# RNG65536/CUDA-volpath

Measured on AMD Instinct MI355X. Metric: Msamples/sec (WxHxspp) + achieved HBM GB/s, Julia 256^3 @ 800x600, higher is better.
Workload: dtype f32; 1 GPU; julia256_800x600_global_majorant; image=800x600, estimator=global_majorant, bound_brick=1, rng=philox2x32-7, parallelism=pixel-tiles x1

## Files before the change

cuda-volpath_amd/csrc/vp_device.h:

```cpp
#pragma once
#include <hip/hip_runtime.h>
#include <stdint.h>

#include "vp_math.h"

namespace vp
{
struct f3 { float x, y, z; };
VP_ARITH_BEGIN
__device__ __forceinline__ f3 mk3(float x, float y, float z) { return f3{x, y, z}; }
__device__ __forceinline__ f3 operator+(f3 a, f3 b) { return f3{a.x + b.x, a.y + b.y, a.z + b.z}; }
__device__ __forceinline__ f3 operator-(f3 a, f3 b) { return f3{a.x - b.x, a.y - b.y, a.z - b.z}; }
__device__ __forceinline__ f3 operator*(f3 a, f3 b) { return f3{a.x * b.x, a.y * b.y, a.z * b.z}; }
__device__ __forceinline__ f3 operator*(f3 a, float s) { return f3{a.x * s, a.y * s, a.z * s}; }
__device__ __forceinline__ f3 operator/(f3 a, float s) { return f3{a.x / s, a.y / s, a.z / s}; }
__device__ __forceinline__ float dot(f3 a, f3 b) { return a.x * b.x + a.y * b.y + a.z * b.z; }
__device__ __forceinline__ f3 cross(f3 a, f3 b)
{
    return f3{a.y * b.z - a.z * b.y, a.z * b.x - a.x * b.z, a.x * b.y - a.y * b.x};
}
__device__ __forceinline__ f3 normalize(f3 v) { return v * rsqrt_(dot(v, v)); }
__device__ __forceinline__ f3 normalize_ieee(f3 v) { return v * (1.0f / __builtin_sqrtf(dot(v, v))); }
__device__ __forceinline__ float max3(f3 v) { return fmaxf(fmaxf(v.x, v.y), v.z); }
__device__ __forceinline__ float min3(f3 v) { return fminf(fminf(v.x, v.y), v.z); }
VP_ARITH_END

#define VP_PI_F 3.1415926535897932384626422832795028841971f
constexpr float kPi     = VP_PI_F;
constexpr float kPi2    = VP_PI_F / 2.0f;
constexpr float k1Pi    = 1.0f / VP_PI_F;
constexpr float k1TwoPi = 1.0f / (VP_PI_F * 2.0f);
constexpr float kTwoPi  = VP_PI_F * 2.0f;
constexpr float k1TwoPiPi = 1.0f / VP_PI_F / (VP_PI_F * 2.0f);

struct ParamDev
{
    unsigned width, height;
    float    density, brightness;
    float    albedo[3];
    float    g;
    float    sigma_t[3];
};

struct SceneDev
{
    const uint2*         cells_u8;
    const float*         cells_f32;
    const unsigned char* bounds_u8;
    const float*         bounds_f32;
    const float*         opacity;
    const float*         opacity_cells;
    const float4*        env;
    int   nx, ny, nz, linear;
    int   cell_bricks;
    int   brick_shift, bnx, bny, bnz;
    int   env_w, env_h;
    float bmin[3], bmax[3], linv[3];
    float sun_dir[3], sun_power[3], sun_orig[3];
    float sun_cos;
    float cam[12];
    float cam_z;
    const float* env_cdf_y;
    const float* env_cdf_x;
    float        env_pdfnorm_alt;
};

__host__ __device__ __forceinline__ unsigned wang_hash(unsigned seed)
{
    seed = (seed ^ 61u) ^ (seed >> 16);
    seed *= 9u;
    seed = seed ^ (seed >> 4);
    seed *= 0x27d4eb2du;
    seed = seed ^ (seed >> 15);
    return seed;
}

struct RngSamplerH
{
    unsigned sx, sy;
    __device__ __forceinline__ void init(unsigned px, unsigned py, unsigned frame, unsigned, unsigned)
    {
        sx = wang_hash((px << 16) | py);
        sy = wang_hash(frame);
        word();
    }
    __device__ __forceinline__ unsigned word()
    {
        unsigned result = sx * 0x9e3779bbu;
        sy ^= sx;
        sx = ((sx << 26) | (sx >> 6)) ^ sy ^ (sy << 9);
        sy = (sx << 13) | (sx >> 19);
        return result;
    }
    __device__ __forceinline__ float next() { return u2f(0x3f800000u | (word() >> 9)) - 1.0f; }
    __device__ __forceinline__ float next_a() { return next(); }
    __device__ __forceinline__ float next_b() { return next(); }
    __device__ __forceinline__ void skip(unsigned n) { for (unsigned i = 0; i < n; i++) word(); }
    static constexpr bool kShadowSubstream = false;
    __device__ __forceinline__ unsigned enter_shadow(unsigned) { return 0u; }
    __device__ __forceinline__ void leave_shadow(unsigned) {}
    __device__ __forceinline__ void set_pair(unsigned) {}
    __device__ __forceinline__ void save(unsigned& a, unsigned& b) const { a = sx; b = sy; }
    __device__ __forceinline__ void load(unsigned a, unsigned b) { sx = a; sy = b; }
};

template <int ROUNDS>
struct RngPhiloxR
{
    unsigned pix, key, pair;
    unsigned w1;
    __device__ __forceinline__ void init(unsigned px, unsigned py, unsigned frame, unsigned key0, unsigned key1)
    {
        pix = (px << 16) | py; key = (frame ^ key0) + key1; pair = 0; w1 = 0;
    }
    __device__ __forceinline__ float next_a()
    {
        unsigned c0 = pair, c1 = pix, k = key;
#pragma unroll
        for (int r = 0; r < ROUNDS; r++)
        {
            unsigned long long p = (unsigned long long)0xD256D193u * c0;
            unsigned n0 = __builtin_amdgcn_bitop3_b32((unsigned)(p >> 32), k, c1, 0x96);
            c1 = (unsigned)p;
            c0 = n0;
            k += 0x9E3779B9u;
        }
        w1 = c1;
        pair++;
        return u2f(0x3f800000u | (c0 >> 9)) - 1.0f;
    }
    __device__ __forceinline__ float next_b() { return u2f(0x3f800000u | (w1 >> 9)) - 1.0f; }
    __device__ __forceinline__ void skip(unsigned n) { pair += n; }
    static constexpr bool kShadowSubstream = true;
    __device__ __forceinline__ unsigned enter_shadow(unsigned id) { const unsigned saved = pair; pair = 0x80000000u + (id << 20); return saved; }
    __device__ __forceinline__ void leave_shadow(unsigned saved) { pair = saved; }
    __device__ __forceinline__ void set_pair(unsigned n) { pair = n; }
    __device__ __forceinline__ void save(unsigned& a, unsigned& b) const { a = pair; b = 0u; }
    __device__ __forceinline__ void load(unsigned a, unsigned) { pair = a; }
};
typedef RngPhiloxR<10> RngPhilox;
typedef RngPhiloxR<7>  RngPhilox7;

VP_ARITH_BEGIN
#define VP_U8_TRI_SCALE 2.3374372e-10f
#define VP_U8_SCALE 0.003921569f

__device__ __forceinline__ f3 to_local(const SceneDev& S, f3 pos)
{
    return f3{(pos.x - S.bmin[0]) * S.linv[0], (pos.y - S.bmin[1]) * S.linv[1], (pos.z - S.bmin[2]) * S.linv[2]};
}

__device__ __forceinline__ void axis_linear(float pn, int n, int& i, float& fw)
{
    float xb = fma_(pn, (float)n, -0.5f);
    xb       = __builtin_fmaxf(xb, 0.0f);
    float fl = __builtin_floorf(xb);
    float fr = xb - fl;
    i        = (int)fl;
    fw       = __builtin_floorf(fma_(fr, 256.0f, 0.5f)) * (1.0f / 256.0f);
    i = i > n - 1 ? n - 1 : i;
}
__device__ __forceinline__ void axis_linear_f32(float pn, int n, int& i, float& fw, bool& low)
{
    float xb = fma_(pn, (float)n, -0.5f);
    float fl = __builtin_floorf(xb);
    float fr = xb - fl;
    i        = (int)fl;
    fw       = __builtin_floorf(fma_(fr, 256.0f, 0.5f)) * (1.0f / 256.0f);
    low      = i < 0;
    i        = i < 0 ? 0 : i;
    i        = i > n - 1 ? n - 1 : i;
}
__device__ __forceinline__ int axis_point(float pn, int n)
{
    int i = (int)__builtin_floorf(pn * (float)n);
    i     = i < 0 ? 0 : i;
    i     = i > n - 1 ? n - 1 : i;
    return i;
}

__device__ __forceinline__ float lerpf(float a, float b, float w) { return a * (1.0f - w) + b * w; }

__device__ __forceinline__ float filter_texels_u8(float t000, float t100, float t010, float t110, float t001, float t101, float t011, float t111,
                                                  float fx, float fy, float fz)
{
    float x00  = fma_(t100 - t000, fx, t000);
    float x10  = fma_(t110 - t010, fx, t010);
    float x01  = fma_(t101 - t001, fx, t001);
    float x11  = fma_(t111 - t011, fx, t011);
    float y0   = fma_(x10 - x00, fy, x00);
    float y1   = fma_(x11 - x01, fy, x01);
    float v    = fma_(y1 - y0, fz, y0);
    return v * (VP_U8_TRI_SCALE * 16777216.0f);
}
__device__ __forceinline__ float filter_cell_u8(uint2 c, float fx, float fy, float fz)
{
    float t000 = (float)(c.x & 0xffu), t100 = (float)((c.x >> 8) & 0xffu);
    float t010 = (float)((c.x >> 16) & 0xffu), t110 = (float)(c.x >> 24);
    float t001 = (float)(c.y & 0xffu), t101 = (float)((c.y >> 8) & 0xffu);
    float t011 = (float)((c.y >> 16) & 0xffu), t111 = (float)(c.y >> 24);
    float x00  = fma_(t100 - t000, fx, t000);
    float x10  = fma_(t110 - t010, fx, t010);
    float x01  = fma_(t101 - t001, fx, t001);
    float x11  = fma_(t111 - t011, fx, t011);
    float y0   = fma_(x10 - x00, fy, x00);
    float y1   = fma_(x11 - x01, fy, x01);
    float v    = fma_(y1 - y0, fz, y0);
    return v * (VP_U8_TRI_SCALE * 16777216.0f);
}

__device__ __forceinline__ size_t cell_index(const SceneDev& S, int i, int j, int k)
{
    if (S.cell_bricks)
    {
        const unsigned nbx = ((unsigned)S.nx + 3u) >> 2, nby = ((unsigned)S.ny + 3u) >> 2;
        const unsigned b   = ((unsigned)i >> 2) + nbx * (((unsigned)j >> 2) + nby * ((unsigned)k >> 2));
        return ((size_t)b << 6) | (size_t)((((unsigned)k & 3u) << 4) | (((unsigned)j & 3u) << 2) | ((unsigned)i & 3u));
    }
    return (size_t)((unsigned)i + __umul24((unsigned)S.nx, (unsigned)j + __umul24((unsigned)S.ny, (unsigned)k)));
}

template <bool QUANT>
__device__ __forceinline__ float sample_density01(const SceneDev& S, f3 pos)
{
    f3    p = to_local(S, pos);
    int   i, j, k;
    float fx, fy, fz;
    bool  lx = false, ly = false, lz = false;
    if (S.linear)
    {
        if (QUANT)
        {
            axis_linear(p.x, S.nx, i, fx);
            axis_linear(p.y, S.ny, j, fy);
            axis_linear(p.z, S.nz, k, fz);
        }
        else
        {
            axis_linear_f32(p.x, S.nx, i, fx, lx);
            axis_linear_f32(p.y, S.ny, j, fy, ly);
            axis_linear_f32(p.z, S.nz, k, fz, lz);
// ... 330 lines not shown
```

cuda-volpath_amd/csrc/vp_integrator.h:

```cpp
enum : int
{
    ST_DONE    = 0,
    ST_SETUP   = 1,
    ST_TRACK   = 2,
    ST_SHADOW  = 3,
    EV_SCATTER = 4,
    EV_NEE     = 5,
    EV_BG      = 6,
    EV_WRITE   = 7,
    EV_MIS     = 8,
    EV_HG      = 9
};

#ifndef VP_PAD_STEP
#define VP_PAD_STEP 0
#endif
#ifndef VP_PAD_FETCH
#define VP_PAD_FETCH 0
#endif
#ifndef VP_PAD_EOF
#define VP_PAD_EOF 0
#endif
#ifndef VP_PAD_SETUP
#define VP_PAD_SETUP 0
// ... 77 lines not shown
    const float c  = Ps + Pn;
    return Ps == 0.0f && sigma_t_prime * wdiv_(inv_sigma_t * c, Pn) == 1.0f;
}

__global__ void light_identity_k(ParamDev P, int local, const unsigned* mask, unsigned* flag)
{
    const unsigned b = threadIdx.x;
    if (local && !(mask[b >> 5] >> (b & 31u) & 1u)) return;
    if (!local && b) return;
    const float max_sig = max3(f3{P.sigma_t[0], P.sigma_t[1], P.sigma_t[2]});
    const float s       = hyperion_s(0 - 5);
    float sigma_t_prime;
    if (local)
    {
        const float reduction   = (1.0f - s) + s * (1.0f - P.g);
        const float cur_density = reduction * P.density;
        const float d_max       = fmaxf(0.0001f, (float)b * VP_U8_SCALE);
        sigma_t_prime           = max_sig * cur_density * d_max;
    }
    else
    {
        const float cur_density = (1.0f - s) * P.density + s * P.density * (1.0f - P.g);
        sigma_t_prime           = max_sig * cur_density;
    }
    const float inv_sigma_t = rcp_(sigma_t_prime);
    if (!(null_collision_in_empty_space(1.0f, sigma_t_prime, inv_sigma_t) == 1.0f)) atomicAnd(flag, 0u);
}

#ifndef VP_LOCAL_MIN_WAVES
#define VP_LOCAL_MIN_WAVES 6
#endif
constexpr int render_min_waves(int est, bool count, int ldsb, bool ach, bool mis, int trk, bool light, bool cancel)
{
    if (VP_MIN_WAVES > 1) return VP_MIN_WAVES;
    if (light) return count ? 5 : (est != EST_GLOBAL ? VP_LIGHT_LOCAL_MIN_WAVES : VP_LIGHT_MIN_WAVES);
    if (mis || ldsb == 1) return 1;
    if (count) return 4;
    if (est == EST_GLOBAL && trk == 0) return VP_GLOBAL_MIN_WAVES;
    if (trk) return 4;
    return (ach && !cancel) ? VP_LOCAL_MIN_WAVES : 5;
}
template <int EST, class RNG, bool QUANT, bool COUNT, int LDSB, bool ACH, bool MIS, int TRK, bool LIGHT = false, bool CANCEL = false>
__global__ __launch_bounds__(LDSB == 1 ? VP_BLOCK_LDS : VP_BLOCK, render_min_waves(EST, COUNT, LDSB, ACH, MIS, TRK, LIGHT, CANCEL))
void render_k(SceneDev S, LaunchDev L)
{
    __shared__ unsigned short lds_bounds[LDSB == 1 ? VP_LDS_BOUND_ENTRIES : 1];
    __shared__ unsigned lds_codes[LDSB == 2 ? VP_LDS_BOUND_ENTRIES / 16 : 1];
    if (LDSB == 2)
    {
        const uint4* src = reinterpret_cast<const uint4*>(L.bound_codes);
        uint4*       dst = reinterpret_cast<uint4*>(lds_codes);
        const int    n16 = (S.bnx * S.bny * S.bnz + 63) / 64;
        for (int w = threadIdx.x; w < n16; w += VP_BLOCK) dst[w] = src[w];
        __syncthreads();
    }
    if (LDSB == 1)
    {
        const uint4* src = reinterpret_cast<const uint4*>(S.bounds_u8);
        uint4*       dst = reinterpret_cast<uint4*>(lds_bounds);
        const int    n16 = (S.bnx * S.bny * S.bnz * 2 + 15) / 16;
        for (int w = threadIdx.x; w < n16; w += VP_BLOCK_LDS) dst[w] = src[w];
        __syncthreads();
    }
    constexpr unsigned KARG_L_   = ((sizeof(SceneDev) + alignof(LaunchDev) - 1) / alignof(LaunchDev)) * alignof(LaunchDev);
    constexpr unsigned KARG_WDS_ = (KARG_L_ + sizeof(LaunchDev) + 3) / 4;
    __shared__ __attribute__((aligned(16))) unsigned kargs_lds_[KARG_WDS_];
    {
        const unsigned* src = (const unsigned*)__builtin_amdgcn_kernarg_segment_ptr();
        for (unsigned w = threadIdx.x; w < KARG_WDS_; w += (LDSB == 1 ? VP_BLOCK_LDS : VP_BLOCK)) kargs_lds_[w] = src[w];
    }
    constexpr bool LOCAL = EST != EST_GLOBAL;
    constexpr bool TAB = TRK == 0 && LDSB != 1 && !LIGHT && !MIS;
    __shared__ __attribute__((aligned(16))) float coll_tab_[TAB ? VP_COLL_ROWS : 1][CR_WORDS];
    if (TAB && threadIdx.x < VP_COLL_ROWS)
        coll_row_fill(coll_tab_[threadIdx.x], (int)threadIdx.x, L.P.g, L.P.density, max3(f3{L.P.sigma_t[0], L.P.sigma_t[1], L.P.sigma_t[2]}), LOCAL);
    __syncthreads();
    auto coll_row = [&](int n) __attribute__((always_inline)) -> const float* {
        return TAB ? coll_tab_[n < 0 ? 0 : (n > VP_COLL_ROWS - 1 ? VP_COLL_ROWS - 1 : n)] : nullptr;
    };
    constexpr bool EARLY = RNG::kShadowSubstream && !MIS && !LIGHT;
    constexpr bool APPR = EST == EST_GLOBAL && TRK == 0 && !LIGHT && !MIS;
    constexpr bool APPR_L = EST == EST_DECOMP && TRK == 0 && !LIGHT && !MIS;
    constexpr bool EXITC = TRK == 0 && !MIS && !LIGHT && EST != EST_BOUNDED && (QUANT || EST == EST_GLOBAL);
    const ParamDev& P = L.P;
    const f3    sig_t     = f3{P.sigma_t[0], P.sigma_t[1], P.sigma_t[2]};
    const f3    sig_s     = sig_t * f3{P.albedo[0], P.albedo[1], P.albedo[2]};
    const float max_sig   = max3(sig_t);
    const float min_sig   = min3(sig_t);
    const float density   = P.density;

    int      st = ST_DONE;
    bool     exhausted = false;
    constexpr bool COLD = LDSB != 1 && !LIGHT;
    constexpr int  CS_  = COLD ? VP_BLOCK : 1;
    static_assert(!COLD || (LOCAL ? VP_LOCAL_MIN_WAVES : VP_GLOBAL_MIN_WAVES) * (14 * VP_BLOCK * 4 + KARG_WDS_ * 4 + VP_COLL_ROWS * CR_WORDS * 4 + (LDSB == 2 ? VP_LDS_BOUND_ENTRIES / 4 : 0)) <= VP_LDS_BYTES_PER_CU,
                  "cold per-path state: more workgroups per CU than the LDS holds -- lower VP_*_MIN_WAVES for this ARCH");
    __shared__ float cold_[COLD ? 14 : 1][CS_];
    float* const cold_p = &cold_[0][COLD ? threadIdx.x : 0];
    ColdF3<COLD, CS_>       rad(cold_p), pd(cold_p + 3 * CS_);
    ColdVal<float, COLD>    ph(cold_p + 6 * CS_), phase_g(cold_p + 7 * CS_);
    ColdVal<unsigned, COLD> item(cold_p + 8 * CS_);
    ColdVal<unsigned, COLD> px(cold_p + 9 * CS_), py(cold_p + 10 * CS_);
    ColdVal<int, COLD>      frame(cold_p + 11 * CS_);
    ColdVal<int, COLD>      nsc(cold_p + 12 * CS_);
    ColdVal<unsigned, COLD> rng_saved(cold_p + 13 * CS_);
    if (COLD) { rad = f3{0.0f, 0.0f, 0.0f}; pd = f3{0.0f, 0.0f, 0.0f}; ph = 0.0f; phase_g = 0.0f; item = 0u; px = 0u; py = 0u; frame = 0; nsc = 0; rng_saved = 0u; }
    RNG      rng;
    f3       ro = {}, rd = {};
    f3       inv_rd = {};
    f3       thr = {};
    int      seg = 0;
    float    dist = 0, t_end = 0;
    float    t_far = 0, distc = 0, inv_sigma = 0, inv_sigma_t = 0, sigma_t_prime = 0, sigma_c = 0;
    float    cur_density = 0, d_max = 0;
    f3       nee_a = {};
    int      terms = 0;
    f3       nee_c = {}, nee_t = {}, seg_o = {};
    int      nee_stage = 0;
    float    sh_inv_sigma = 0, sh_density = 0;
    float    sig_base = density;
    int      chan = 0;
    float    t_empty = 0.0f;
    float    t_clip = 1e30f;
    bool     ex_clear = false;
    unsigned long long c_load = 0, c_xtest = 0, c_xout = 0, c_xok = 0;
    unsigned zrun = 0;

    unsigned long long c_den = 0, c_bnd = 0, c_opa = 0, c_env = 0, c_sca = 0, c_smp = 0;
    unsigned long long d_iter = 0, d_act = 0, d_outer = 0, d_shadow = 0;
    constexpr bool PROF = COUNT && VP_PROFILE_BLOCKS;
    unsigned long long t_slow = 0, t_fast = 0, t_mark = PROF ? __builtin_amdgcn_s_memtime() : 0ull;
    enum { B_SETUP, B_HALF, B_LOOK, B_EXIT, B_SCATTER, B_NEE, B_HG, B_BG, B_WRITE, B_REFILL, B_GSETUP, B_FETCH, B_ZERO, B_ZERO_SH, B_EXITT, B_NBLK };
    unsigned long long bw[B_NBLK] = {}, bl[B_NBLK] = {};
    unsigned long long hist[3][8] = {};
    unsigned long long ctrl_w = 0, ctrl_l = 0;
    auto tally = [&](int b, bool on) __attribute__((always_inline)) {
        if (PROF)
        {
            unsigned long long m = __ballot(on);
            if (m)
            {
                bw[b] += 1; bl[b] += (unsigned)__popcll(m);
                const int h = b == B_SCATTER ? 0 : b == B_EXIT ? 1 : b == B_SETUP ? 2 : -1;
                if (h >= 0) hist[h][((unsigned)__popcll(m) - 1u) >> 3] += 1;
            }
        }
    };

    const unsigned lane = threadIdx.x & 63u;
    unsigned chunk_s = 0, chunk_n = 0;
    unsigned chunk_q = 0, chunk_f0 = 0;
    bool     queue_empty = false;
    unsigned q_cur   = __builtin_amdgcn_s_getreg((4 - 1) << 11 | 20) & (VP_NQUEUES - 1);
    unsigned q_tried = 0;
    unsigned end_skipped = 0;
    unsigned visits = 0;

    for (;;)
    {
        if (PROF && lane == 0) d_outer++;
        {
#ifdef VP_EXP_FLAT_KARGS
        const char* kargs_ = (const char*)__builtin_amdgcn_kernarg_segment_ptr();
        asm volatile("" : "+s"(kargs_));
#else
        unsigned ko_ = 0;
        asm volatile("" : "+v"(ko_));
        const char* kargs_ = reinterpret_cast<const char*>(kargs_lds_) + ko_;
#endif
        const SceneDev&  S = *reinterpret_cast<const SceneDev*>(kargs_);
        const LaunchDev& L = *reinterpret_cast<const LaunchDev*>(kargs_ + KARG_L_);
        const ParamDev&  P = L.P;
        const f3 sun_dir   = f3{S.sun_dir[0], S.sun_dir[1], S.sun_dir[2]};
        const f3 sun_power = f3{S.sun_power[0], S.sun_power[1], S.sun_power[2]};
        auto start_shadow = [&](f3 end, float inv_s, float den, unsigned stage) __attribute__((always_inline)) {
            f3    sd = normalize(end - ro);
            float tn, tf;
            bool  hitv = intersect_box(ro, sd, S, tn, tf);
            if (!hitv)
            {
                nee_a = f3{1.0f, 1.0f, 1.0f};
                st    = EV_NEE;
            }
            else
            {
                if (tn < 0.0f) tn = 0.0f;
                f3 se       = ro - end;
                t_end       = fminf(tf, sqrt_(dot(se, se)));
                dist        = tn;
                terms       = 0;
                rd          = sd;
                inv_sigma   = inv_s;
                cur_density = den;
                st          = ST_SHADOW;
                rng_saved = rng.enter_shadow(2u * (unsigned)(int)nsc + stage);
                if (COUNT) t_clip = 1e30f;
                if (RNG::kShadowSubstream && stage == 0u && L.sun_clip)
                {
                    f3    pl = to_local(S, ro);
                    int   ci, cj, ck;
                    float w_;
                    axis_linear(pl.x, S.nx, ci, w_);
                    axis_linear(pl.y, S.ny, cj, w_);
                    axis_linear(pl.z, S.nz, ck, w_);
                    const unsigned n = L.sun_clip[(size_t)((unsigned)ci + __umul24((unsigned)S.nx, (unsigned)cj + __umul24((unsigned)S.ny, (unsigned)ck)))];
                    if (n != 0xffffu)
                    {
                        const float tc = (float)n * L.clip_ds;
                        if (COUNT && !L.count_clips) t_clip = tc;
                        else t_end = fminf(t_end, tc);
                    }
                }
            }
        };
        auto segment_medium = [&]() __attribute__((always_inline)) {
            if (LOCAL && TAB) cur_density = coll_row(nsc - 5)[CR_DENS];
            else if (LOCAL)
            {
                float s         = hyperion_s(nsc - 5);
                phase_g         = (1.0f - s) * P.g;
                float reduction = (1.0f - s) + s * (1.0f - P.g);
                cur_density     = TRK ? reduction * sig_base : reduction * density;
            }
        };
        auto next_segment = [&]() __attribute__((always_inline)) {
            st = ST_SETUP;
            if (LOCAL) dist = -1.0f;
            if (EXITC) terms = L.exit_start;
            if (EST == EST_GLOBAL) nsc = nsc + 1;
            if (EST == EST_BOUNDED) seg++;
            if ((EST == EST_BOUNDED ? seg : nsc) >= 800) st = EV_WRITE;
            segment_medium();
        };
        auto finish_light = [&]() __attribute__((always_inline)) {
            rad = rad + sun_power * (((ACH ? f3{thr.x, thr.x, thr.x} : thr) * ph) * nee_a);
            rd  = pd;
            next_segment();
        };
        tally(B_SCATTER, st == EV_SCATTER);
        if (!LIGHT && st == EV_SCATTER)
        {
            vp_pad<VP_PAD_COLL>();
            if (COUNT) c_sca++;
            if (PROF) zrun = 0;
            t_empty = 0.0f;
            if (LOCAL) nsc = nsc + 1;
            const int          n2   = LOCAL ? (nsc - 5) : (nsc - 4);
            const float* const row2 = coll_row(n2);
            const float* const rowp = coll_row(n2 - 1);
            float s2 = hyperion_s(n2);
            float dp2, stp2;
            if (TAB)
            {
                dp2  = row2[CR_DENS];
                stp2 = LOCAL ? row2[CR_STP] * d_max : row2[CR_STP];
            }
            else if (TRK)
            {
                thr  = thr * f3{P.albedo[0], P.albedo[1], P.albedo[2]};
                stp2 = LOCAL ? ((1.0f - s2) + s2 * (1.0f - P.g)) * sig_base : (1.0f - s2) * sig_base + s2 * sig_base * (1.0f - P.g);
                dp2  = stp2;
            }
            else if (LOCAL)
            {
                float reduction2 = (1.0f - s2) + s2 * (1.0f - P.g);
                dp2              = reduction2 * density;
                stp2             = max_sig * dp2 * d_max;
            }
            else
            {
                dp2  = (1.0f - s2) * density + s2 * density * (1.0f - P.g);
                stp2 = max_sig * dp2;
            }
            ph = TAB ? hg_eval_row(rowp, dot(rd, sun_dir)) : hg_eval(phase_g, dot(rd, sun_dir));
            pd = rd;
            if (EARLY)
            {
                Frame fr(rd);
                float r0 = rng.next_a();
                float r1 = rng.next_b();
                pd       = normalize(fr.to_world(TAB ? hg_sample_local_row(rowp, r0, r1) : hg_sample_local(phase_g, r0, r1)));
                if (LOCAL) { const f3 pdv = pd; inv_rd = f3{rcp_(pdv.x), rcp_(pdv.y), rcp_(pdv.z)}; }
            }
            if (MIS)
            {
                sh_inv_sigma = rcp_(stp2);
                sh_density   = dp2;
                nee_stage    = 0;
                nee_c        = sun_power;
                nee_t        = (ACH ? f3{thr.x, thr.x, thr.x} : thr) * ph;
            }
            if (EST == EST_DECOMP && frame > 10 && nsc > 20)
            {
                float op = sample_float_cells(S, S.opacity_cells, ro);
                if (COUNT) c_opa++;
                if (TRK)
                {
                    float a = expf_(-stp2 * op);
                    nee_a   = f3{a, a, a};
                }
                else if (ACH)
                {
                    float a = expf_(((-sig_t.x) * dp2) * op);
                    nee_a   = f3{a, a, a};
                }
                else
                {
                    f3 tau = (f3{-sig_t.x, -sig_t.y, -sig_t.z} * dp2) * op;
                    nee_a  = f3{expf_(tau.x), expf_(tau.y), expf_(tau.z)};
                }
                st     = EV_NEE;
                if (EARLY) finish_light();
            }
            else
            {
                start_shadow(sun_dir * 1e10f, (TAB && !LOCAL) ? row2[CR_INV] : rcp_(stp2), dp2, 0u);
                if (EARLY && st == EV_NEE) finish_light();
                if (EARLY && EST == EST_GLOBAL && st == ST_SHADOW)
                {
                    float tn2, tf2;
                    bool  hit2 = intersect_box(ro, pd, S, tn2, tf2);
                    t_empty    = tn2 < 0.0f ? 0.0f : tn2;
                    t_far      = hit2 ? tf2 : -1.0f;
                    if (TAB) { sigma_t_prime = row2[CR_STP]; inv_sigma_t = row2[CR_INV]; }
                }
            }
        }
#pragma unroll
        for (int pass = 0; pass < (MIS ? 2 : 1); pass++)
        {
            tally(B_NEE, st == EV_NEE);
            if (!LIGHT && !EARLY && st == EV_NEE)
            {
                if (MIS)
                {
                    rad = rad + nee_c * (nee_t * nee_a);
                    st  = nee_stage == 0 ? EV_MIS : EV_HG;
                }
                else
                {
                    rad = rad + sun_power * (((ACH ? f3{thr.x, thr.x, thr.x} : thr) * ph) * nee_a);
                    st  = EV_HG;
                }
            }
            if (MIS && st == EV_MIS)
            {
                const float P_phase = 0.5f, P_envmap = 1.0f - P_phase;
                const f3    thr3    = ACH ? f3{thr.x, thr.x, thr.x} : thr;
                Frame       fr(pd);
                nee_stage = 1;
                if (rng.next_a() < P_phase)
                {
                    float u        = rng.next_a();
                    float v        = rng.next_b();
                    f3    brdf_dir = fr.to_world(hg_sample_local(phase_g, u, v));
                    f3    envc     = eval_envmap(S, brdf_dir);
                    if (COUNT) c_env++;
                    float pdf_brdf        = hg_eval(phase_g, dot(fr.n, brdf_dir));
                    float pdf_env_virtual = luminance(envc) * S.env_pdfnorm_alt;
                    float wa = pdf_brdf * P_phase, wb = pdf_env_virtual * P_envmap;
                    float weight = wa / (wa + wb) / P_phase;
                    nee_c = envc;
                    nee_t = thr3 * weight;
                    start_shadow(brdf_dir * 1e10f, sh_inv_sigma, sh_density, 1u);
                }
                else
                {
                    float u = rng.next_a();
                    float v = rng.next_b();
                    f3    envc;
                    float pdf_env = sample_envmap(S, u, v, envc);
                    if (COUNT) c_env++;
                    if (pdf_env <= 0.0f)
// ... 299 lines not shown
ends_done:
        if (CANCEL && L.cancel && (visits++ & 7u) == 0u)
        {
            unsigned w = 0;
            if (lane == 0) w = __hip_atomic_load(L.cancel, __ATOMIC_RELAXED, __HIP_MEMORY_SCOPE_AGENT);
            if ((unsigned)__builtin_amdgcn_readfirstlane((int)w) >= L.batch_id) { st = ST_DONE; exhausted = true; queue_empty = true; }
        }
        if (__ballot(st != ST_DONE || !exhausted) == 0ull) break;
        }
        if (PROF) { unsigned long long t = __builtin_amdgcn_s_memtime(); if (lane == 0) t_slow += t - t_mark; t_mark = t; }

        auto segment_setup = [&]() __attribute__((always_inline)) {
            if (LOCAL) tally(B_SETUP, st == ST_SETUP);
            if (LOCAL && st == ST_SETUP)
            {
                vp_pad<VP_PAD_SETUP>();
                float t_near, tf;
                bool  hit = intersect_box_inv(ro, inv_rd, S, t_near, tf);
                t_near    = fmaxf(t_near, 0.0f);
                t_far     = fminf(tf, 0.05f);
                float bx, by;
                if (LDSB)
                {
                    f3  pl = to_local(S, ro + rd * t_near);
                    int bi = axis_point(pl.x, S.nx) >> S.brick_shift;
                    int bj = axis_point(pl.y, S.ny) >> S.brick_shift;
                    int bk = axis_point(pl.z, S.nz) >> S.brick_shift;
                    const unsigned bidx = (unsigned)bi + __umul24((unsigned)S.bnx, (unsigned)bj + __umul24((unsigned)S.bny, (unsigned)bk));
                    unsigned v;
                    if (LDSB == 2)
                    {
                        const unsigned code = (lds_codes[bidx >> 4] >> ((bidx & 15u) << 1)) & 3u;
                        const unsigned pal  = (code & 2u) ? L.bound_pal[1] : L.bound_pal[0];
                        v = (code & 1u) ? pal >> 16 : pal & 0xffffu;
                    }
                    else
                        v = lds_bounds[bidx];
                    bx = (float)(v & 0xffu) * VP_U8_SCALE;
                    by = (float)(v >> 8) * VP_U8_SCALE;
                }
                else
                    sample_bound<QUANT>(S, ro + rd * t_near, bx, by);
                if (COUNT) c_bnd++;
                float d_min = by;
                d_max       = fmaxf(0.0001f, bx);
                if (!hit) st = EV_BG;
                else
                {
                    dist          = fmaxf(dist, t_near);
                    sigma_t_prime = TRK ? cur_density : max_sig * cur_density * d_max;
                    inv_sigma_t   = rcp_(sigma_t_prime);
                    if (PROF)
                    {
                        const unsigned long long cm = __ballot(TRK == 0 && EST == EST_DECOMP && d_min > 0.0f);
                        if (cm) { ctrl_w += 1; ctrl_l += (unsigned)__popcll(cm); }
                    }
                    if (TRK == 0 && EST == EST_DECOMP && d_min > 0.0f)
                    {
                        sigma_c       = min_sig * cur_density * d_min;
                        distc         = dist - div_(logf_(rng.next_a()), fmaxf(sigma_c, 1e-20f));
                        float sigma_r = fmaxf(sigma_t_prime - sigma_c, 1e-20f);
                        inv_sigma     = rcp_(sigma_r);
                    }
                    else
                    {
                        distc     = 1e20f;
                        sigma_c   = 0.0f;
                        inv_sigma = inv_sigma_t;
                    }
                    t_end = fminf(distc, t_far);
                    st    = ST_TRACK;
                }
            }
        };
        auto light_done = [&]() __attribute__((always_inline)) {
#ifdef VP_EXP_FLAT_KARGS
            const char* ka_ = (const char*)__builtin_amdgcn_kernarg_segment_ptr();
            asm volatile("" : "+s"(ka_));
#else
            unsigned ko2_ = 0;
            asm volatile("" : "+v"(ko2_));
            const char* ka_ = reinterpret_cast<const char*>(kargs_lds_) + ko2_;
#endif
            const SceneDev& S2 = *reinterpret_cast<const SceneDev*>(ka_);
            const f3 sunp = f3{S2.sun_power[0], S2.sun_power[1], S2.sun_power[2]};
            rad = rad + sunp * (((ACH ? f3{thr.x, thr.x, thr.x} : thr) * ph) * nee_a);
            rd  = pd;
            if (EXITC) terms = reinterpret_cast<const LaunchDev*>(ka_ + KARG_L_)->exit_start;
            if (EST == EST_GLOBAL)
            {
                nsc = nsc + 1;
                if (nsc >= 800) st = EV_WRITE;
                else if (t_far < 0.0f) { st = EV_BG; t_empty = 0.0f; }
                else
                {
                    t_end         = t_far;
                    dist          = t_empty;
                    t_empty       = 0.0f;
                    float s       = hyperion_s(nsc - 5);
                    if (!TAB) phase_g = (1.0f - s) * P.g;
                    if (TAB)
                    {
                    }
                    else if (TRK)
                    {
                        sigma_t_prime = (1.0f - s) * sig_base + s * sig_base * (1.0f - P.g);
                        cur_density   = sigma_t_prime;
                    }
                    else
                    {
                        cur_density   = (1.0f - s) * density + s * density * (1.0f - P.g);
                        sigma_t_prime = max_sig * cur_density;
                    }
                    if (!TAB)
                    {
                        inv_sigma   = rcp_(sigma_t_prime);
                        inv_sigma_t = inv_sigma;
                    }
                    st            = ST_TRACK;
                }
            }
            else
            {
                st   = ST_SETUP;
                dist = -1.0f;
                if (EST == EST_BOUNDED) seg++;
                if ((EST == EST_BOUNDED ? seg : nsc) >= 800) st = EV_WRITE;
                if (TAB) cur_density = coll_row(nsc - 5)[CR_DENS];
                else
                {
                    float s         = hyperion_s(nsc - 5);
                    phase_g         = (1.0f - s) * P.g;
                    float reduction = (1.0f - s) + s * (1.0f - P.g);
                    cur_density     = TRK ? reduction * sig_base : reduction * density;
                }
            }
        };
        auto tracking_step = [&]() __attribute__((always_inline)) {
            tally(B_HALF, st == ST_TRACK || st == ST_SHADOW);
            if (LIGHT && !LOCAL)
            {
                if (st == ST_TRACK)
                {
                    dist += -logf_(rng.next_a()) * inv_sigma;
                    if (dist >= t_end) st = EV_BG;
                    else
                    {
                        (void)rng.next_b();
                        if (COUNT) c_den++;
                        seg++;
                    }
                }
                return;
            }
            if (st == ST_TRACK || st == ST_SHADOW)
            {
                const bool shadow = st == ST_SHADOW;
                vp_pad<VP_PAD_STEP>();
                dist += -logf_(rng.next_a()) * inv_sigma;
                tally(B_EXIT, dist >= t_end || (shadow && terms == 7));
                tally(B_LOOK, !(dist >= t_end || (shadow && terms == 7)));
                if (dist >= t_end || (shadow && terms == 7))
                {
                    vp_pad<VP_PAD_EOF>();
                    if (shadow)
                    {
                        nee_a = f3{(float)(1 - (terms & 1)), (float)(1 - ((terms >> 1) & 1)), (float)(1 - ((terms >> 2) & 1))};
                        st    = EV_NEE;
                        rng.leave_shadow(rng_saved);
                        if (EARLY) light_done();
                    }
                    else if (LOCAL)
                    {
                        bool through = fminf(distc, dist) >= t_far;
                        if (through)
                        {
                            ro = ro + rd * t_far;
                            t_empty -= t_far;
                            st   = ST_SETUP;
                            dist = -1.0f;
                            if (EXITC) terms += d_max <= 0.0001f ? VP_EXIT_TRIP : 0;
                            if (EST == EST_BOUNDED && ++seg >= 800) st = EV_WRITE;
                        }
                        else
                        {
                            if (MIS) seg_o = ro;
                            ro = ro + rd * distc;
                            st = LIGHT ? EV_WRITE : EV_SCATTER;
                        }
                    }
                    else
                    {
                        st = EV_BG;
                        if (PROF) { c_xout += zrun; zrun = 0; }
                    }
                }
                else
                {
                    vp_pad<VP_PAD_FETCH>();
                    f3    p   = ro + rd * dist;
                    float den;
                    tally(B_FETCH, !LIGHT && (shadow || !(dist < t_empty)));
                    if (LIGHT) den = 0.0f;
                    else if (EST == EST_GLOBAL)
                    {
                        den = 0.0f;
                        if (shadow || !(dist < t_empty))
                        {
                            den = sample_density01<QUANT>(S, p) * cur_density;
                            if (COUNT && !(shadow && dist >= t_clip) && !(!shadow && ex_clear)) c_load++;
                        }
                    }
                    else
                    {
                        den = 0.0f;
                        if (shadow || !(dist < t_empty))
                        {
                            den = sample_density01<QUANT>(S, p) * cur_density;
                            if (COUNT && !(shadow && dist >= t_clip) && !(!shadow && ex_clear)) c_load++;
                        }
                    }
                    float e   = rng.next_b();
                    if (COUNT) c_den++;
                    tally(B_ZERO, !LIGHT && !shadow && !(dist < t_empty) && den == 0.0f);
                    tally(B_ZERO_SH, !LIGHT && shadow && den == 0.0f && !(COUNT && dist >= t_clip));
                    if (TRK)
                    {
                        if (e < den * inv_sigma)
                        {
                            if (shadow) { nee_a = f3{0.0f, 0.0f, 0.0f}; st = EV_NEE; rng.leave_shadow(rng_saved); if (EARLY) light_done(); }
                            else { ro = p; st = EV_SCATTER; }
                        }
                    }
                    else if (shadow)
                    {
                        if (ACH) terms = (e < sig_t.x * den * inv_sigma) ? 7 : terms;
                        else
                        {
                            int t = terms;
                            t |= (e < sig_t.x * den * inv_sigma) ? 1 : 0;
                            t |= (e < sig_t.y * den * inv_sigma) ? 2 : 0;
                            t |= (e < sig_t.z * den * inv_sigma) ? 4 : 0;
                            terms = t;
                        }
                    }
                    else if (ACH)
                    {
                        float a_t = sig_t.x * den, a_s = sig_s.x * den;
                        if (LOCAL) { a_t = a_t - sigma_c; a_s = a_s - sigma_c; }
                        float a_n  = sigma_t_prime - a_t;
                        float mt   = __builtin_fabsf(a_t * thr.x), mn = __builtin_fabsf(a_n * thr.x);
                        float Ps   = (mt + mt) + mt;
                        float Pn   = (mn + mn) + mn;
                        float c    = Ps + Pn;
                        bool  real = e * c < Ps;
                        float f    = wdiv_(inv_sigma_t * c, real ? Ps : Pn);
                        thr.x      = thr.x * ((real ? a_s : a_n) * f);
                        if (real)
                        {
                            if (MIS) seg_o = ro;
                            ro = p;
                            st = LIGHT ? EV_WRITE : EV_SCATTER;
                        }
                        else if (EXITC && den == 0.0f)
                        {
                            terms++;
                            if (PROF) zrun++;
                        }
                    }
                    else
                    {
                        f3 sigma_t_den = sig_t * den;
                        f3 sigma_s_den = sig_s * den;
                        if (LOCAL)
                        {
                            f3 sc       = f3{sigma_c, sigma_c, sigma_c};
                            sigma_t_den = sigma_t_den - sc;
                            sigma_s_den = sigma_s_den - sc;
                        }
                        f3    sigma_null_den = f3{sigma_t_prime, sigma_t_prime, sigma_t_prime} - sigma_t_den;
                        float Ps = __builtin_fabsf(sigma_t_den.x * thr.x) + __builtin_fabsf(sigma_t_den.y * thr.y) +
                                   __builtin_fabsf(sigma_t_den.z * thr.z);
                        float Pn = __builtin_fabsf(sigma_null_den.x * thr.x) + __builtin_fabsf(sigma_null_den.y * thr.y) +
                                   __builtin_fabsf(sigma_null_den.z * thr.z);
                        float c    = Ps + Pn;
                        bool  real = e * c < Ps;
                        float f    = wdiv_(inv_sigma_t * c, real ? Ps : Pn);
                        f3    sel  = real ? sigma_s_den : sigma_null_den;
                        thr        = thr * (sel * f);
                        if (real)
                        {
                            if (MIS) seg_o = ro;
                            ro = p;
                            st = LIGHT ? EV_WRITE : EV_SCATTER;
                        }
                        else if (EXITC && den == 0.0f)
                        {
                            terms++;
                            if (PROF) zrun++;
                        }
                    }
                }
            }
        };
        constexpr int STEPS = (LIGHT && !LOCAL) ? VP_LIGHT_STEPS_PER_PASS : VP_STEPS_PER_PASS;
#pragma unroll 1
        for (int iter = 0;; iter += STEPS)
        {
            bool active = (st == ST_TRACK) || (st == ST_SHADOW) || (LOCAL && st == ST_SETUP);
            unsigned long long am = __ballot(active);
            unsigned long long wm = __ballot(!active && !(st == ST_DONE && exhausted));
            unsigned nwait = (unsigned)__popcll(wm);
            if (am == 0ull || nwait >= L.wait_lanes || (nwait > 0u && iter >= (int)L.wait_iters)) break;
            if (PROF)
            {
                const unsigned long long sm = __ballot(st == ST_SHADOW);
                if (lane == 0) { d_iter++; d_act += (unsigned)__popcll(am); d_shadow += (unsigned)__popcll(sm); }
            }
            if (!active) continue;
            segment_setup();
            tracking_step();
#pragma unroll
            for (int u = 1; u < STEPS; u++)
            {
                if (PROF)
                {
                    unsigned long long am2 = __ballot((st == ST_TRACK) || (st == ST_SHADOW) || (LOCAL && st == ST_SETUP));
                    const unsigned long long sm2 = __ballot(st == ST_SHADOW);
                    if (lane == 0) { d_iter++; d_act += (unsigned)__popcll(am2); d_shadow += (unsigned)__popcll(sm2); }
                }
                if (LOCAL && (unsigned)__popcll(__ballot(st == ST_SETUP)) >= L.setup_lanes) segment_setup();
                tracking_step();
            }
        }
        if (PROF) { unsigned long long t = __builtin_amdgcn_s_memtime(); if (lane == 0) t_fast += t - t_mark; t_mark = t; }
    }

    if (COUNT)
    {
        unsigned long long vals[12] = {c_smp, c_den, c_bnd, c_opa, c_env, c_sca, d_iter, d_act, d_outer, d_shadow, t_slow, t_fast};
#pragma unroll
        for (int q = 0; q < (PROF ? 12 : 6); q++)
        {
            unsigned long long v = vals[q];
            for (int off = 32; off > 0; off >>= 1) v += __shfl_down(v, off, 64);
            if (lane == 0) atomicAdd(&L.counters[q], v);
        }
        {
            unsigned long long v = c_load;
            for (int off = 32; off > 0; off >>= 1) v += __shfl_down(v, off, 64);
            if (lane == 0) atomicAdd(&L.counters[12], v);
        }
        {
            unsigned long long xv[3] = {c_xtest, c_xout, c_xok};
#pragma unroll
            for (int q = 0; q < 3; q++)
            {
                unsigned long long v = xv[q];
                for (int off = 32; off > 0; off >>= 1) v += __shfl_down(v, off, 64);
                if (lane == 0) atomicAdd(&L.counters[13 + q], v);
            }
        }
        if (PROF && lane == 0)
        {
#pragma unroll
            for (int b = 0; b < B_NBLK; b++) { atomicAdd(&L.counters[16 + 2 * b], bw[b]); atomicAdd(&L.counters[17 + 2 * b], bl[b]); }
#pragma unroll
            for (int h = 0; h < 3; h++)
#pragma unroll
                for (int q = 0; q < 8; q++) atomicAdd(&L.counters[48 + 8 * h + q], hist[h][q]);
            atomicAdd(&L.counters[72], ctrl_w); atomicAdd(&L.counters[73], ctrl_l);
        }
    }
}

__device__ __forceinline__ bool approach_cancelled(const LaunchDev& L)
// ... 203 lines not shown
```

Measured before the change: 3294 Msamples/s.

## Defer NEE light accumulation via LDS cold state and park scatter position

Shadow-ray results are now stored as a termination bitmask plus a pre-multiplied light weight in LDS cold slots. The radiance add is applied later at the next scatter instead of being computed at shadow exit, which drops the live nee_a/ph registers and the kernarg sun_power reload in the hot loop. The scatter position is also parked as a distance and applied once at the scatter event rather than updated on every collision. Smaller tweaks replace floor with fract/truncation in axis_linear and use alignbit for the RNG float conversion. The extra cold slots add LDS per block, and bookkeeping for deferred results must stay correct across path ends.

```diff
diff --git a/cuda-volpath_amd/csrc/vp_device.h b/cuda-volpath_amd/csrc/vp_device.h
--- a/cuda-volpath_amd/csrc/vp_device.h
+++ b/cuda-volpath_amd/csrc/vp_device.h
@@ -75,6 +75,11 @@
     return seed;
 }
 
+__device__ __forceinline__ float draw_to_float(unsigned w)
+{
+    return u2f(__builtin_amdgcn_alignbit(0x7fu, w, 9u)) - 1.0f;
+}
+
 struct RngSamplerH
 {
     unsigned sx, sy;
@@ -127,9 +132,9 @@
         }
         w1 = c1;
         pair++;
-        return u2f(0x3f800000u | (c0 >> 9)) - 1.0f;
-    }
-    __device__ __forceinline__ float next_b() { return u2f(0x3f800000u | (w1 >> 9)) - 1.0f; }
+        return draw_to_float(c0);
+    }
+    __device__ __forceinline__ float next_b() { return draw_to_float(w1); }
     __device__ __forceinline__ void skip(unsigned n) { pair += n; }
     static constexpr bool kShadowSubstream = true;
     __device__ __forceinline__ unsigned enter_shadow(unsigned id) { const unsigned saved = pair; pair = 0x80000000u + (id << 20); return saved; }
@@ -154,9 +159,8 @@
 {
     float xb = fma_(pn, (float)n, -0.5f);
     xb       = __builtin_fmaxf(xb, 0.0f);
-    float fl = __builtin_floorf(xb);
-    float fr = xb - fl;
-    i        = (int)fl;
+    float fr = __builtin_amdgcn_fractf(xb);
+    i        = (int)xb;
     fw       = __builtin_floorf(fma_(fr, 256.0f, 0.5f)) * (1.0f / 256.0f);
     i = i > n - 1 ? n - 1 : i;
 }
diff --git a/cuda-volpath_amd/csrc/vp_integrator.h b/cuda-volpath_amd/csrc/vp_integrator.h
--- a/cuda-volpath_amd/csrc/vp_integrator.h
+++ b/cuda-volpath_amd/csrc/vp_integrator.h
@@ -183,6 +183,8 @@
     constexpr bool APPR = EST == EST_GLOBAL && TRK == 0 && !LIGHT && !MIS;
     constexpr bool APPR_L = EST == EST_DECOMP && TRK == 0 && !LIGHT && !MIS;
     constexpr bool EXITC = TRK == 0 && !MIS && !LIGHT && EST != EST_BOUNDED && (QUANT || EST == EST_GLOBAL);
+    constexpr bool PARK = !MIS;
+    constexpr bool DEFER = EARLY && TRK == 0;
     const ParamDev& P = L.P;
     const f3    sig_t     = f3{P.sigma_t[0], P.sigma_t[1], P.sigma_t[2]};
     const f3    sig_s     = sig_t * f3{P.albedo[0], P.albedo[1], P.albedo[2]};
@@ -194,9 +196,10 @@
     bool     exhausted = false;
     constexpr bool COLD = LDSB != 1 && !LIGHT;
     constexpr int  CS_  = COLD ? VP_BLOCK : 1;
-    static_assert(!COLD || (LOCAL ? VP_LOCAL_MIN_WAVES : VP_GLOBAL_MIN_WAVES) * (14 * VP_BLOCK * 4 + KARG_WDS_ * 4 + VP_COLL_ROWS * CR_WORDS * 4 + (LDSB == 2 ? VP_LDS_BOUND_ENTRIES / 4 : 0)) <= VP_LDS_BYTES_PER_CU,
+    constexpr int NCOLD = 14 + (DEFER ? (ACH ? 1 : 3) : 0);
+    static_assert(!COLD || (LOCAL ? VP_LOCAL_MIN_WAVES : VP_GLOBAL_MIN_WAVES) * (NCOLD * VP_BLOCK * 4 + KARG_WDS_ * 4 + VP_COLL_ROWS * CR_WORDS * 4 + (LDSB == 2 ? VP_LDS_BOUND_ENTRIES / 4 : 0)) <= VP_LDS_BYTES_PER_CU,
                   "cold per-path state: more workgroups per CU than the LDS holds -- lower VP_*_MIN_WAVES for this ARCH");
-    __shared__ float cold_[COLD ? 14 : 1][CS_];
+    __shared__ float cold_[COLD ? NCOLD : 1][CS_];
     float* const cold_p = &cold_[0][COLD ? threadIdx.x : 0];
     ColdF3<COLD, CS_>       rad(cold_p), pd(cold_p + 3 * CS_);
     ColdVal<float, COLD>    ph(cold_p + 6 * CS_), phase_g(cold_p + 7 * CS_);
@@ -205,7 +208,11 @@
     ColdVal<int, COLD>      frame(cold_p + 11 * CS_);
     ColdVal<int, COLD>      nsc(cold_p + 12 * CS_);
     ColdVal<unsigned, COLD> rng_saved(cold_p + 13 * CS_);
+    constexpr unsigned LIGHT_NONE = 0xffffffffu;
+    ColdVal<float, COLD>    lw_x(cold_p + 6 * CS_), lw_y(cold_p + (DEFER && !ACH ? 14 : 6) * CS_), lw_z(cold_p + (DEFER && !ACH ? 15 : 6) * CS_);
+    ColdVal<unsigned, COLD> light_bits(cold_p + (DEFER ? NCOLD - 1 : 6) * CS_);
     if (COLD) { rad = f3{0.0f, 0.0f, 0.0f}; pd = f3{0.0f, 0.0f, 0.0f}; ph = 0.0f; phase_g = 0.0f; item = 0u; px = 0u; py = 0u; frame = 0; nsc = 0; rng_saved = 0u; }
+    if (DEFER) { lw_x = 0.0f; if (!ACH) { lw_y = 0.0f; lw_z = 0.0f; } light_bits = LIGHT_NONE; }
     RNG      rng;
     f3       ro = {}, rd = {};
     f3       inv_rd = {};
@@ -334,16 +341,29 @@
             segment_medium();
         };
         auto finish_light = [&]() __attribute__((always_inline)) {
-            rad = rad + sun_power * (((ACH ? f3{thr.x, thr.x, thr.x} : thr) * ph) * nee_a);
+            if (DEFER) rad = rad + sun_power * ((ACH ? f3{lw_x, lw_x, lw_x} : f3{lw_x, lw_y, lw_z}) * nee_a);
+            else rad = rad + sun_power * (((ACH ? f3{thr.x, thr.x, thr.x} : thr) * ph) * nee_a);
             rd  = pd;
             next_segment();
         };
+        if (DEFER)
+        {
+            const unsigned lb = light_bits;
+            if (lb != LIGHT_NONE)
+            {
+                const int tb = (int)lb;
+                const f3  na = f3{(float)(1 - (tb & 1)), (float)(1 - ((tb >> 1) & 1)), (float)(1 - ((tb >> 2) & 1))};
+                rad          = rad + sun_power * ((ACH ? f3{lw_x, lw_x, lw_x} : f3{lw_x, lw_y, lw_z}) * na);
+                light_bits   = LIGHT_NONE;
+            }
+        }
         tally(B_SCATTER, st == EV_SCATTER);
         if (!LIGHT && st == EV_SCATTER)
         {
             vp_pad<VP_PAD_COLL>();
             if (COUNT) c_sca++;
             if (PROF) zrun = 0;
+            if (PARK) ro = ro + rd * dist;
             t_empty = 0.0f;
             if (LOCAL) nsc = nsc + 1;
             const int          n2   = LOCAL ? (nsc - 5) : (nsc - 4);
@@ -373,7 +393,13 @@
                 dp2  = (1.0f - s2) * density + s2 * density * (1.0f - P.g);
                 stp2 = max_sig * dp2;
             }
-            ph = TAB ? hg_eval_row(rowp, dot(rd, sun_dir)) : hg_eval(phase_g, dot(rd, sun_dir));
+            const float phv = TAB ? hg_eval_row(rowp, dot(rd, sun_dir)) : hg_eval(phase_g, dot(rd, sun_dir));
+            if (DEFER)
+            {
+                lw_x = thr.x * phv;
+                if (!ACH) { lw_y = thr.y * phv; lw_z = thr.z * phv; }
+            }
+            else ph = phv;
             pd = rd;
             if (EARLY)
             {
@@ -389,7 +415,7 @@
                 sh_density   = dp2;
                 nee_stage    = 0;
                 nee_c        = sun_power;
-                nee_t        = (ACH ? f3{thr.x, thr.x, thr.x} : thr) * ph;
+                nee_t        = (ACH ? f3{thr.x, thr.x, thr.x} : thr) * phv;
             }
             if (EST == EST_DECOMP && frame > 10 && nsc > 20)
             {
@@ -855,9 +881,13 @@
             asm volatile("" : "+v"(ko2_));
             const char* ka_ = reinterpret_cast<const char*>(kargs_lds_) + ko2_;
 #endif
-            const SceneDev& S2 = *reinterpret_cast<const SceneDev*>(ka_);
-            const f3 sunp = f3{S2.sun_power[0], S2.sun_power[1], S2.sun_power[2]};
-            rad = rad + sunp * (((ACH ? f3{thr.x, thr.x, thr.x} : thr) * ph) * nee_a);
+            if (DEFER) light_bits = (unsigned)terms;
+            else
+            {
+                const SceneDev& S2 = *reinterpret_cast<const SceneDev*>(ka_);
+                const f3 sunp = f3{S2.sun_power[0], S2.sun_power[1], S2.sun_power[2]};
+                rad = rad + sunp * (((ACH ? f3{thr.x, thr.x, thr.x} : thr) * ph) * nee_a);
+            }
             rd  = pd;
             if (EXITC) terms = reinterpret_cast<const LaunchDev*>(ka_ + KARG_L_)->exit_start;
             if (EST == EST_GLOBAL)
@@ -938,7 +968,7 @@
                     vp_pad<VP_PAD_EOF>();
                     if (shadow)
                     {
-                        nee_a = f3{(float)(1 - (terms & 1)), (float)(1 - ((terms >> 1) & 1)), (float)(1 - ((terms >> 2) & 1))};
+                        if (!DEFER) nee_a = f3{(float)(1 - (terms & 1)), (float)(1 - ((terms >> 1) & 1)), (float)(1 - ((terms >> 2) & 1))};
                         st    = EV_NEE;
                         rng.leave_shadow(rng_saved);
                         if (EARLY) light_done();
@@ -958,7 +988,8 @@
                         else
                         {
                             if (MIS) seg_o = ro;
-                            ro = ro + rd * distc;
+                            if (PARK) dist = distc;
+                            else ro = ro + rd * distc;
                             st = LIGHT ? EV_WRITE : EV_SCATTER;
                         }
                     }
@@ -1002,7 +1033,7 @@
                         if (e < den * inv_sigma)
                         {
                             if (shadow) { nee_a = f3{0.0f, 0.0f, 0.0f}; st = EV_NEE; rng.leave_shadow(rng_saved); if (EARLY) light_done(); }
-                            else { ro = p; st = EV_SCATTER; }
+                            else { if (!PARK) ro = p; st = EV_SCATTER; }
                         }
                     }
                     else if (shadow)
@@ -1032,7 +1063,7 @@
                         if (real)
                         {
                             if (MIS) seg_o = ro;
-                            ro = p;
+                            if (!PARK) ro = p;
                             st = LIGHT ? EV_WRITE : EV_SCATTER;
                         }
                         else if (EXITC && den == 0.0f)
@@ -1064,7 +1095,7 @@
                         if (real)
                         {
                             if (MIS) seg_o = ro;
-                            ro = p;
+                            if (!PARK) ro = p;
                             st = LIGHT ? EV_WRITE : EV_SCATTER;
                         }
                         else if (EXITC && den == 0.0f)
```

Result: faster. 3436 Msamples/s (median of 6 runs) (+4.3%).
